# wljungbergh/mpc-trajectory-generator

Measured on AMD Instinct MI355X. Metric: nmpc_solves_per_sec, higher is better.
Workload: dtype f64

## Files before the change

### mpc_trajectory_generator_amd/csrc/nmpc_kernels.hip

```cpp
#include "nmpc_device.h"
#include "../../include/nmpc_solver.h"

#include <cfloat>
#include <cstdio>
#include <cstdlib>
#include <cstring>
#include <memory>
#include <string>
#include <vector>

#include "nmpc_layout.h"
#include "nmpc_probe.h"
#include "nmpc_eval.h"
#include "nmpc_solve_common.h"
#include "nmpc_solve_hyb.h"
#include "nmpc_solve_hyb2.h"
#include "nmpc_rng.h"
#include "nmpc_loop.h"
#include "nmpc_plan.h"
#include "nmpc_order.h"
#include "nmpc_host.h"

using nmpc::DevBuf;
using nmpc::Event;
// ... 18 lines not shown
    SOLVE_ROW(nmpc_solve_hyb_kernel, 20, Timed<ShapeNobs50>),
    SOLVE_ROW(nmpc_solve_hyb_kernel, 20, Timed<ShapeAny>),
    SOLVE_ROW(nmpc_solve_hyb2_kernel, 40, ShapeN40),
    SOLVE_ROW(nmpc_solve_hyb2_kernel, 40, ShapeAny),
    SOLVE_ROW(nmpc_solve_hyb2_kernel, 40, Timed<ShapeN40>),
    SOLVE_ROW(nmpc_solve_hyb2_kernel, 40, Timed<ShapeAny>),
};
#undef SOLVE_ROW
}
using nmpc::SolveKernel;

struct Staging {
    DevBuf<double> p, u, y0, c0, yout, psi, grad, F1, F2;
    DevBuf<nmpc_status> st;
    PinBuf pin[2];
    Event ev[2];
    bool ready = false;
};
struct SmallArena {
    DevBuf<char> d;
    PinBuf h;
    Event ev[2];
    bool ready = false;
    void release() { *this = {}; }
};
struct Pools {
    DevBuf<double> park;
    DevBuf<int> pool;
    DevBuf<unsigned int> ctr;
    bool made() const { return park && pool && ctr; }
    void release() { *this = {}; }
};

struct nmpc_handle {
    nmpc_problem pb{};
    nmpc_opts op{};
    int device = 0;
    int max_batch = 0;
    bool alive = true;
    LdsMap map{};
    int P = 20;
    const SolveKernel *kernel[2] = {nullptr, nullptr};
    int grid_cap = 0;
    double last_ms = 0.0;
    size_t team_lds = 0;
    size_t eval_lds = 0;
    DevBuf<unsigned int> d_queue;
    int park_min = 500, park_depth = 8;
    int sched_mode = 1;
    double sched_theta = 0.0, sched_cold = 0.4;
    bool shape_any = false;
    int team_owners_forced = 0;
    bool team_help = true;
    int waves_per_cu = 0;
    int dbg = 0;
    double cull_radius = 0.0;
    Pools pools;
    bool loop_order_prev = true;
    DevBuf<int> d_order;
    bool use_order = true;
    DevBuf<unsigned char> d_cls;
    Staging stg;
    SmallArena small;
    double tl_dur_ms = 0.0, tl_budget_ms = 0.0;
    long long tl_dur = 0, tl_budget = 0;
    DevBuf<long long> d_t0;
    std::string err;
};

__global__ void nmpc_stamp_kernel(long long *t0)
{
    if (threadIdx.x == 0) *t0 = (long long)__builtin_amdgcn_s_memrealtime();
}

extern "C" {

void nmpc_default_opts(nmpc_opts *o)
{
    o->tolerance = 1e-4;
    o->initial_tolerance = 1e-4;
    o->delta_tolerance = 1e-4;
    o->initial_penalty = 1.0;
    o->penalty_update = 5.0;
    o->tolerance_update = 0.1;
    o->sufficient_decrease = 0.1;
    o->lbfgs_memory = 10;
    o->max_inner = 500;
    o->max_outer = 10;
    o->max_total_inner = 0;
    o->akkt_gradient = 1;
    o->ls_failure = 0;
    o->inner_status = 0;
    o->reserved = 0;
}

int nmpc_n_u(const nmpc_problem *pb) { return 2 * pb->N; }
int nmpc_n1(const nmpc_problem *pb) { return 2 * pb->N; }
int nmpc_n2(const nmpc_problem *pb) { return pb->nobs + pb->ndyn; }
int nmpc_n_p(const nmpc_problem *pb) { return nmpc::NZ + pb->N + 3 * pb->nobs + 5 * pb->ndyn * pb->N + 3 * pb->N; }
int nmpc_abi_version(void) { return NMPC_ABI_VERSION; }
int nmpc_experiments_build(void)
{
#ifdef NMPC_EXPERIMENTS
    return 1;
#else
    return 0;
#endif
}

static int fail(nmpc_handle *h, int code, const char *what, hipError_t e = hipSuccess)
{
    if (h) {
        h->err = what;
        if (e != hipSuccess) { h->err += ": "; h->err += hipGetErrorString(e); }
    }
    return code;
}

#define HIP_TRY(h, call)                                                       \
    do {                                                                       \
        hipError_t e_ = (call);                                                \
        if (e_ != hipSuccess) return fail((h), NMPC_ERR_HIP, #call, e_);       \
    } while (0)

static constexpr size_t LDS_PER_CU = 160 * 1024;
static LdsMap make_map(const nmpc_problem &pb, int P) { return nmpc::lds_layout(pb.N, pb.nobs, pb.ndyn, P); }

static void read_knobs([[maybe_unused]] nmpc_handle *h)
{
#ifdef NMPC_EXPERIMENTS
    auto ival = [](const char *name, int &v) { if (const char *e = getenv(name)) v = atoi(e); };
    auto flag = [](const char *name, bool &v) { if (const char *e = getenv(name)) v = atoi(e) != 0; };
    auto pos = [](const char *name, double &v) { if (const char *e = getenv(name)) { const double x = atof(e); if (x > 0.0) v = x; } };
    if (const char *e = getenv("NMPC_SHAPE")) h->shape_any = !strcmp(e, "any");
    ival("NMPC_PARK_MIN", h->park_min);
    ival("NMPC_PARK_DEPTH", h->park_depth);
    flag("NMPC_LOOP_ORDER_PREV", h->loop_order_prev);
    ival("NMPC_SCHED", h->sched_mode);
    pos("NMPC_SCHED_THETA", h->sched_theta);
    pos("NMPC_SCHED_COLD", h->sched_cold);
    pos("NMPC_CULL_RADIUS", h->cull_radius);
    flag("NMPC_TEAM_HELP", h->team_help);
    flag("NMPC_ORDER", h->use_order);
    int owners = 0; ival("NMPC_TEAM_OWNERS", owners);
    if (owners >= 1 && owners <= nmpc::TEAM_WAVES) h->team_owners_forced = owners;
    ival("NMPC_WAVES_PER_CU", h->waves_per_cu);
    ival("NMPC_DEBUG_PRIO", h->dbg);
#endif
}

int nmpc_new(const nmpc_problem *pb, const nmpc_opts *opts, int device_id, int max_batch, nmpc_handle **out)
{
    if (!pb || !out || max_batch < 1) return NMPC_ERR_BAD_ARG;
    if (pb->N < 2 || pb->N > NMPC_MAX_HORIZON || pb->nobs < 0 || pb->nobs > 64 || pb->ndyn < 0 || pb->ndyn > nmpc::NDYN_MAX)
        return NMPC_ERR_BAD_PROBLEM;
    auto finite = [](double x) { return x >= -DBL_MAX && x <= DBL_MAX; };
    if (!(pb->ts > 0.0 && pb->ts <= DBL_MAX) || !finite(pb->vmin) || !finite(pb->vmax) || !(pb->vmin <= pb->vmax) ||
        !finite(pb->amin) || !finite(pb->amax) || !(pb->amin <= pb->amax) ||
        !(pb->wmax >= 0.0 && pb->wmax <= DBL_MAX) || !(pb->awmax >= 0.0 && pb->awmax <= DBL_MAX))
        return NMPC_ERR_BAD_PROBLEM;
    nmpc_opts op;
    if (opts) op = *opts; else nmpc_default_opts(&op);
    if (op.lbfgs_memory < 1 || op.lbfgs_memory > nmpc::MAXMEM || op.max_inner < 1 || op.max_outer < 1 ||
        op.max_total_inner < 0 || op.akkt_gradient < 0 || op.akkt_gradient > 2 || op.ls_failure < 0 || op.ls_failure > 1 ||
        op.inner_status < 0 || op.inner_status > 1)
        return NMPC_ERR_BAD_OPTS;
    auto finite_pos = [](double x) { return x > 0.0 && x <= DBL_MAX; };
    if (!finite_pos(op.tolerance) || !finite_pos(op.initial_tolerance) || !finite_pos(op.delta_tolerance) ||
        !(op.initial_tolerance >= op.tolerance) || !finite_pos(op.initial_penalty) ||
        !(op.penalty_update > 1.0 && op.penalty_update <= DBL_MAX) ||
        !(op.tolerance_update > 0.0 && op.tolerance_update < 1.0) ||
        !(op.sufficient_decrease > 0.0 && op.sufficient_decrease < 1.0))
        return NMPC_ERR_BAD_OPTS;
    int ndev = 0;
    if (hipGetDeviceCount(&ndev) != hipSuccess || ndev <= 0 || device_id < 0 || device_id >= ndev)
        return NMPC_ERR_NO_DEVICE;
    nmpc_handle *h = new nmpc_handle();
    h->pb = *pb; h->op = op; h->device = device_id; h->max_batch = max_batch;
    h->P = pb->N <= 20 ? 20 : 40;
    h->map = make_map(*pb, h->P == 40 ? 64 : h->P);
    h->sched_theta = h->P == 20 ? 0.5 : 0.8;
    h->cull_radius = 1.1 * pb->N * pb->ts * fmax(fabs(pb->vmin), fabs(pb->vmax));
    read_knobs(h);
    for (const SolveKernel &k : nmpc::SOLVE_KERNELS)
        if (k.P == h->P && (k.N == 0 ? !h->kernel[k.timed] : !h->shape_any && k.N == pb->N && k.nobs == pb->nobs && k.ndyn == pb->ndyn))
            h->kernel[k.timed] = &k;
    const size_t slice = (size_t)(h->P == 40 ? nmpc::lds_layout2(pb->N, pb->nobs, pb->ndyn).total : h->map.total) * sizeof(double);
    h->eval_lds = 3 * slice;
    h->team_lds = nmpc::TEAM_WAVES * slice + nmpc::TEAM_CTL_INTS * sizeof(int);
    if (h->eval_lds > LDS_PER_CU || h->team_lds > LDS_PER_CU) { nmpc_free(h); return NMPC_ERR_BAD_PROBLEM; }
    hipDeviceProp_t prop;
    hipError_t e = hipSetDevice(device_id);
    (void)hipGetDeviceProperties(&prop, device_id);
    if (e == hipSuccess) e = h->d_queue.alloc(1);
    if (e == hipSuccess) e = h->d_order.alloc(max_batch);
// ... 29 lines not shown
    const double t = ceil(ms * 1e5);
    const double cap = 4503599627370496.0;
    return t < 1.0 ? 1 : (long long)(t < cap ? t : cap);
}

int nmpc_set_time_limits(nmpc_handle *h, double max_duration_ms, double batch_budget_ms)
{
    if (!h) return NMPC_ERR_BAD_ARG;
    if (!h->alive) return NMPC_ERR_DEAD_HANDLE;
    auto ok = [](double x) { return x >= 0.0 && x <= DBL_MAX; };
    if (!ok(max_duration_ms) || !ok(batch_budget_ms)) return fail(h, NMPC_ERR_BAD_OPTS, "time limits: negative, NaN or infinite");
    const long long budget = ms_to_ticks(batch_budget_ms);
    if (budget > 0 && !h->d_t0) {
        HIP_TRY(h, hipSetDevice(h->device));
        HIP_TRY(h, h->d_t0.alloc(1));
    }
    h->tl_dur_ms = max_duration_ms; h->tl_budget_ms = batch_budget_ms;
    h->tl_dur = ms_to_ticks(max_duration_ms); h->tl_budget = budget;
    return NMPC_OK;
}

static int check_batch(nmpc_handle *h, int B, const double *p, const double *u)
{
    if (!h) return NMPC_ERR_BAD_ARG;
    if (!h->alive) return NMPC_ERR_DEAD_HANDLE;
    if (B < 0 || B > h->max_batch || (B > 0 && (!p || !u))) return fail(h, NMPC_ERR_BAD_ARG, "bad batch arguments");
    return NMPC_OK;
}

static void fill_args(const nmpc_handle *h, KArgs &a, int B)
{
    std::memset(&a, 0, sizeof(a));
    a.pb = h->pb; a.op = h->op; a.map = h->map; a.B = B;
    a.n_p = nmpc_n_p(&h->pb); a.n_u = nmpc_n_u(&h->pb); a.n1 = nmpc_n1(&h->pb); a.n2 = nmpc_n2(&h->pb);
    a.queue = h->d_queue;
    a.inv_ts = 1.0 / h->pb.ts;
    a.dbg = h->dbg;
    a.tl_dur = h->tl_dur; a.tl_budget = h->tl_budget;
    a.tl_t0 = h->tl_budget > 0 ? h->d_t0.p : nullptr;
}

static int solve_launch(nmpc_handle *h, int B, const double *d_p, double *d_u, const double *d_y0, const double *d_c0, double *d_y_out,
                        nmpc_status *d_status, const nmpc_status *prev, void *stream)
{
    if (const int rc = check_batch(h, B, d_p, d_u); rc || B == 0) return rc;
    hipStream_t s = (hipStream_t)stream;
    HIP_TRY(h, hipSetDevice(h->device));
    KArgs a;
    fill_args(h, a, B);
    a.p = d_p; a.u = d_u; a.y0 = d_y0; a.c0 = d_c0; a.y_out = d_y_out; a.st = d_status;
    if (h->tl_budget > 0) hipLaunchKernelGGL(nmpc_stamp_kernel, dim3(1), dim3(64), 0, s, h->d_t0.p);
    HIP_TRY(h, hipMemsetAsync(h->d_queue, 0, sizeof(unsigned int), s));
    const int grid = B < h->grid_cap ? B : h->grid_cap;
    if (B > grid) {
        if (h->use_order) {
            if (prev) hipLaunchKernelGGL(nmpc::nmpc_classify_prev_kernel, dim3((B + 255) / 256), dim3(256), 0, s, B, prev, h->d_cls.p);
            else hipLaunchKernelGGL(nmpc::nmpc_classify_kernel, dim3((B + 255) / 256), dim3(256), 0, s, a, h->d_cls.p);
            hipLaunchKernelGGL(nmpc::nmpc_order_kernel, dim3(1), dim3(1024), 0, s, B, h->d_cls.p, h->d_order.p);
            a.order = h->d_order;
        }
        if ((h->P == 20 && (h->park_min > 0 || h->sched_mode > 0)) || (h->P == 40 && h->sched_mode > 0)) {
            const size_t cap = (size_t)B;
            const size_t cap_max = (size_t)h->max_batch;
            Pools &pl = h->pools;
            if (!pl.made()) {
                pl.release();
                HIP_TRY(h, pl.park.alloc(cap_max * nmpc::park_stride(h->pb.N)));
                HIP_TRY(h, pl.pool.alloc(nmpc::NPOOLS * cap_max));
                HIP_TRY(h, pl.ctr.alloc(4 * nmpc::NPOOLS + 2));
            }
            HIP_TRY(h, hipMemsetAsync(pl.pool, 0xFF, nmpc::NPOOLS * cap * sizeof(int), s));
            HIP_TRY(h, hipMemsetAsync(pl.ctr, 0, (4 * nmpc::NPOOLS + 2) * sizeof(unsigned int), s));
            a.park_min = h->P == 20 ? h->park_min : 0; a.park_depth = h->park_depth;
            a.park = pl.park; a.pool = pl.pool; a.pool_ctr = pl.ctr; a.pool_cap = (int)cap;
            a.sched_mode = h->sched_mode;
        }
    }
    {
        const int max_wgs = h->grid_cap / nmpc::TEAM_WAVES;
        int owners = (B + max_wgs - 1) / max_wgs;
        if (owners > nmpc::TEAM_WAVES) owners = nmpc::TEAM_WAVES;
        if (h->team_owners_forced > 0) owners = h->team_owners_forced;
        int wgs = (grid + owners - 1) / owners;
        if (wgs > max_wgs) wgs = max_wgs;
        a.team_owners = owners;
        a.sched_long_cap = (int)(h->sched_theta * (double)(wgs * owners));
        a.sched_cold_cap = (int)(h->sched_cold * (double)(wgs * owners));
        a.team_help = h->team_help;
        a.cull_radius = h->cull_radius;
        hipLaunchKernelGGL(h->kernel[timed(h)]->fn, dim3(wgs), dim3(64 * nmpc::TEAM_WAVES), h->team_lds, s, a);
    }
    HIP_TRY(h, hipGetLastError());
    return NMPC_OK;
}

int nmpc_solve_batch_device(nmpc_handle *h, int B, const double *d_p, double *d_u, const double *d_y0,
                            const double *d_c0, double *d_y_out, nmpc_status *d_status, void *stream)
{
    return solve_launch(h, B, d_p, d_u, d_y0, d_c0, d_y_out, d_status, nullptr, stream);
}

int nmpc_eval_batch_device(nmpc_handle *h, int B, const double *d_p, const double *d_u, const double *d_c,
                           const double *d_y, double *d_psi, double *d_grad, double *d_F1, double *d_F2,
                           void *stream)
{
    if (const int rc = check_batch(h, B, d_p, d_u); rc || B == 0) return rc;
    hipStream_t s = (hipStream_t)stream;
    HIP_TRY(h, hipSetDevice(h->device));
    KArgs a;
    fill_args(h, a, B);
    a.p = d_p; a.u = const_cast<double *>(d_u);
    a.ev_c = d_c; a.ev_y = d_y; a.ev_psi = d_psi; a.ev_grad = d_grad; a.ev_F1 = d_F1; a.ev_F2 = d_F2;
    const dim3 grid((B + 2) / 3);
    if (h->P == 40) hipLaunchKernelGGL(nmpc::nmpc_eval2_kernel, grid, dim3(64), h->eval_lds, s, a);
    else hipLaunchKernelGGL(nmpc::nmpc_eval_kernel<20>, grid, dim3(64), h->eval_lds, s, a);
    HIP_TRY(h, hipGetLastError());
    return NMPC_OK;
}

static constexpr size_t PIN_CHUNK = 4u << 20;
static int ensure_staging(nmpc_handle *h)
{
    Staging &g = h->stg;
    if (g.ready) return NMPC_OK;
    if (g.p) return fail(h, NMPC_ERR_HIP, "staging buffers: an earlier allocation failed half way");
    const size_t B = (size_t)h->max_batch;
    const size_t np = nmpc_n_p(&h->pb), nu = nmpc_n_u(&h->pb), n1 = nmpc_n1(&h->pb), n2 = nmpc_n2(&h->pb) + 1;
    HIP_TRY(h, hipSetDevice(h->device));
    HIP_TRY(h, g.p.alloc(B * np));
    HIP_TRY(h, g.u.alloc(B * nu));
    HIP_TRY(h, g.y0.alloc(B * n1));
    HIP_TRY(h, g.c0.alloc(B));
    HIP_TRY(h, g.yout.alloc(B * n1));
    HIP_TRY(h, g.psi.alloc(B));
    HIP_TRY(h, g.grad.alloc(B * nu));
    HIP_TRY(h, g.F1.alloc(B * n1));
    HIP_TRY(h, g.F2.alloc(B * n2));
    HIP_TRY(h, g.st.alloc(B));
    for (int k = 0; k < 2; ++k) {
        HIP_TRY(h, g.pin[k].alloc(PIN_CHUNK));
        HIP_TRY(h, g.ev[k].create(hipEventDisableTiming));
    }
    g.ready = true;
    return NMPC_OK;
// ... 187 lines not shown
```

### mpc_trajectory_generator_amd/csrc/nmpc_layout.h

```cpp
#pragma once

#ifndef NMPC_WIN
#define NMPC_WIN 1
#endif

namespace nmpc {

constexpr int NZ = 20;
constexpr int MAXMEM = 10;
constexpr int NDYN_MAX = 3;
constexpr int GRAM_LD = 11;
constexpr int GRAM_NST = 20;
constexpr int OBS_STRIDE = 4;
constexpr int SEG_STRIDE = 5;
constexpr int TEAM_WAVES = 4;
constexpr int TEAM_REQ_DOUBLES = 3 * 24 * 2;
constexpr int TEAM_AREA_DOUBLES = 3 * 24 * 2 + 8;
constexpr int TEAM_CTL_INTS = 64;
constexpr int NPOOLS = 2;
enum { POOL_LONG = 0, POOL_COLD = 1 };

constexpr double GAMMA_L_COEFF = 0.95;
constexpr double DELTA_LIPSCHITZ = 1e-12;
constexpr double EPSILON_LIPSCHITZ = 1e-6;
constexpr double LIPSCHITZ_UPDATE_EPSILON = 1e-6;
constexpr int MAX_LIPSCHITZ_UPDATE_ITERATIONS = 10;
constexpr double MAX_LIPSCHITZ_CONSTANT = 1e9;
constexpr double MIN_LIPSCHITZ_CONSTANT = 1e-10;
constexpr int MAX_LINESEARCH_ITERATIONS = 10;
constexpr double LBFGS_SY_EPSILON = 1e-10;
constexpr double LBFGS_CBFGS_EPSILON = 1e-8;

struct LdsMap {
    int sc;
    int cw;
    int par;
    int seg;
    int obs;
    int f2;
    int dyn;
    int dyn_stride;
    int req;
    int vec;
    int rho;
    int S, Y;
    int nv;
    int gsy, gyy;
    int total;
};

struct KArgs {
    nmpc_problem pb;
    nmpc_opts op;
    LdsMap map;
    int B;
    int n_p, n_u, n1, n2;
    double inv_ts;
    const double *p;
    double *u;
    const double *y0;
    const double *c0;
    double *y_out;
    nmpc_status *st;
    unsigned int *queue;
    const int *order;
    int park_min;
    int park_depth;
    double *park;
    int *pool;
    unsigned int *pool_ctr;
    int pool_cap;
    int sched_mode;
    int sched_long_cap;
    int sched_cold_cap;
    int dbg;
    int team_owners;
    int team_help;
    double cull_radius;
    union {
        struct {
            const double *ev_c;
            const double *ev_y;
            double *ev_psi, *ev_grad, *ev_F1, *ev_F2;
        };
        struct {
            long long tl_dur;
            long long tl_budget;
            const long long *tl_t0;
        };
    };
};

enum { SC_X0 = 0, SC_Y0, SC_TH0, SC_VINIT, SC_WINIT, SC_XF, SC_YF, SC_THF,
       SC_Q, SC_QV, SC_QTH, SC_RV, SC_RW, SC_QN, SC_QTHN, SC_QCTE, SC_PA, SC_PW };

typedef __attribute__((address_space(3))) double lds_double;
typedef double dbl2 __attribute__((ext_vector_type(2)));
typedef __attribute__((address_space(3))) dbl2 lds_double2;

#ifdef NMPC_NO_SCHED_BARRIER
#define NMPC_SCHED_BARRIER() do { } while (0)
#else
#define NMPC_SCHED_BARRIER() __builtin_amdgcn_sched_barrier(0)
#endif
#define NMPC_WAVE_SYNC()                                           \
    do {                                                           \
        __builtin_amdgcn_fence(__ATOMIC_RELEASE, "workgroup");     \
        __builtin_amdgcn_wave_barrier();                           \
        __builtin_amdgcn_fence(__ATOMIC_ACQUIRE, "workgroup");     \
    } while (0)

enum { DY_EX = 0, DY_EY, DY_CA, DY_SA, DY_IRX2, DY_IRY2, DY_FIELDS };
struct DynStage {
    const lds_double *col;
    int stride;
    __device__ __forceinline__ double get(int k, int f) const { return col[(k * DY_FIELDS + f) * stride]; }
};

struct ShapeAny { static constexpr int N = 0, NOBS = -1, NDYN = -1; };
struct ShapeDefault { static constexpr int N = 20, NOBS = 10, NDYN = 3; };
struct ShapeNobs50 { static constexpr int N = 20, NOBS = 50, NDYN = 3; };
struct ShapeN40 { static constexpr int N = 40, NOBS = 10, NDYN = 3; };
template <class S> struct Timed { static constexpr int N = S::N, NOBS = S::NOBS, NDYN = S::NDYN; };
template <class SH> struct ShapeTimed { static constexpr bool value = false; };
template <class S> struct ShapeTimed<Timed<S>> { static constexpr bool value = true; };
template <class SH> __device__ __forceinline__ int shape_N(const KArgs &a) { if constexpr (SH::N > 0) return SH::N; else return a.pb.N; }
template <class SH> __device__ __forceinline__ int shape_nobs(const KArgs &a) { if constexpr (SH::NOBS >= 0) return SH::NOBS; else return a.pb.nobs; }
template <class SH> __device__ __forceinline__ int shape_ndyn(const KArgs &a) { if constexpr (SH::NDYN >= 0) return SH::NDYN; else return a.pb.ndyn; }

__host__ __device__ constexpr LdsMap lds_layout(int N, int nobs, int ndyn, int P)
// ... 103 lines not shown
```

### mpc_trajectory_generator_amd/csrc/nmpc_solve_hyb.h

```cpp
#pragma once

#ifndef NMPC_CULL_MIN
#define NMPC_CULL_MIN 16
#endif
#ifndef NMPC_WIN
#define NMPC_WIN 1
#endif

namespace nmpc {

typedef __attribute__((address_space(3))) int lds_int;
enum { CTL_OWNERS = 0, CTL_HELPERS = 1, CTL_CLAIM = 4, CTL_DONE = 8, CTL_INST = 56 };
__device__ __forceinline__ int ctl_load(lds_int *p) { return __hip_atomic_load(p, __ATOMIC_RELAXED, __HIP_MEMORY_SCOPE_WORKGROUP); }
__device__ __forceinline__ void ctl_store(lds_int *p, int v) { __hip_atomic_store(p, v, __ATOMIC_RELAXED, __HIP_MEMORY_SCOPE_WORKGROUP); }
__device__ __forceinline__ int ctl_add(lds_int *p, int v) { return __hip_atomic_fetch_add(p, v, __ATOMIC_RELAXED, __HIP_MEMORY_SCOPE_WORKGROUP); }

__device__ __forceinline__ double point_scalar(double v, int k)
{
    const int lo = __builtin_amdgcn_readlane(__double2loint(v), 16 * k);
    const int hi = __builtin_amdgcn_readlane(__double2hiint(v), 16 * k);
    return __hiloint2double(hi, lo);
}

#define NMPC_FETCH_GRAD(K, OV, OW)                                             \
    do {                                                                       \
        const dbl2 fg_ = zgr[(K) * ZS];                                        \
        OV = fg_.x; OW = fg_.y;                                                \
    } while (0)

#define NMPC_HALF_STEP(xv, xw)                                                 \
    do {                                                                       \
        const double s1_ = fma(-gamma, gv, (xv)), s2_ = fma(-gamma, gw, (xw)); \
        hv = ina ? clampd(s1_, vmin, vmax) : s1_;                              \
        hw = ina ? clampd(s2_, -wmax, wmax) : s2_;                             \
    } while (0)
#define NMPC_FBE(xv, xw) fbe_value<P>(cost, gamma, pk_hig, fma(-gamma, gv, (xv)), fma(-gamma, gw, (xw)), hv, hw, gv, gw, lane)

constexpr int POOL_CTRS = 4;
__device__ __forceinline__ int pool_pop(const KArgs &a, int c)
{
    unsigned int *ctr = a.pool_ctr + POOL_CTRS * c;
    int *cnt = (int *)(ctr + 2);
    if (__hip_atomic_load(cnt, __ATOMIC_RELAXED, __HIP_MEMORY_SCOPE_AGENT) <= 0) return -1;
    if (__hip_atomic_fetch_add(cnt, -1, __ATOMIC_RELAXED, __HIP_MEMORY_SCOPE_AGENT) <= 0) {
        __hip_atomic_fetch_add(cnt, 1, __ATOMIC_RELAXED, __HIP_MEMORY_SCOPE_AGENT);
        return -1;
    }
    const unsigned pos = __hip_atomic_fetch_add(&ctr[0], 1u, __ATOMIC_RELAXED, __HIP_MEMORY_SCOPE_AGENT);
    int *slot = a.pool + (size_t)c * a.pool_cap + pos % (unsigned)a.pool_cap;
    int inst;
    do { inst = __hip_atomic_load(slot, __ATOMIC_ACQUIRE, __HIP_MEMORY_SCOPE_AGENT); } while (inst < 0);
    __hip_atomic_store(slot, -1, __ATOMIC_RELAXED, __HIP_MEMORY_SCOPE_AGENT);
    return inst;
}
__device__ __forceinline__ void pool_push(const KArgs &a, int c, int inst)
{
    unsigned int *ctr = a.pool_ctr + POOL_CTRS * c;
    const unsigned pos = __hip_atomic_fetch_add(&ctr[1], 1u, __ATOMIC_RELAXED, __HIP_MEMORY_SCOPE_AGENT);
    int *slot = a.pool + (size_t)c * a.pool_cap + pos % (unsigned)a.pool_cap;
    while (__hip_atomic_load(slot, __ATOMIC_RELAXED, __HIP_MEMORY_SCOPE_AGENT) >= 0) __builtin_amdgcn_s_sleep(1);
    __hip_atomic_store(slot, inst, __ATOMIC_RELEASE, __HIP_MEMORY_SCOPE_AGENT);
    __hip_atomic_fetch_add((int *)(ctr + 2), 1, __ATOMIC_RELEASE, __HIP_MEMORY_SCOPE_AGENT);
}
__device__ __forceinline__ int pool_depth(const KArgs &a, int c)
{
    return __hip_atomic_load((int *)(a.pool_ctr + POOL_CTRS * c + 2), __ATOMIC_RELAXED, __HIP_MEMORY_SCOPE_AGENT);
}

template <int J>
__device__ __forceinline__ double fnma_row_bcast(double acc, double x, double y)
{
    asm("s_nop 1\n\tv_fmac_f64_dpp %0, -%1, %2 row_newbcast:%3 row_mask:0xf bank_mask:0xf" : "+v"(acc) : "v"(x), "v"(y), "n"(J));
    return acc;
}
template <int J>
__device__ __forceinline__ double fma_row_bcast(double acc, double x, double y)
{
    asm("s_nop 1\n\tv_fmac_f64_dpp %0, %1, %2 row_newbcast:%3 row_mask:0xf bank_mask:0xf" : "+v"(acc) : "v"(x), "v"(y), "n"(J));
    return acc;
}
template <int J>
__device__ __forceinline__ void fnma3_row_bcast(double &a1, double &a2, double &a3, double x, double y1, double y2, double y3, double after)
{
    asm("v_fmac_f64_dpp %0, -%3, %4 row_newbcast:%8 row_mask:0xf bank_mask:0xf\n\t"
        "v_fmac_f64_dpp %1, -%3, %5 row_newbcast:%8 row_mask:0xf bank_mask:0xf\n\t"
        "v_fmac_f64_dpp %2, -%3, %6 row_newbcast:%8 row_mask:0xf bank_mask:0xf"
        : "+v"(a1), "+v"(a2), "+v"(a3) : "v"(x), "v"(y1), "v"(y2), "v"(y3), "v"(after), "n"(J));
}
template <int J>
__device__ __forceinline__ void fma2_row_bcast(double &a1, double &a2, double x, double y1, double y2, double after)
{
// ... 166 lines not shown
    lds_double2 *Lgk = Los + 6 * COLS;
    lds_double2 *LypE = (lds_double2 *)(L + mp.vec) + 3 * COLS + te;
    lds_double2 *Ly = (lds_double2 *)(L + mp.vec) + 4 * COLS + te;
    lds_double *Lvr = L + mp.vec + 2 * 5 * COLS + te;
#define NMPC_LB_ZERO()                                                                                  \
    do {                                                                                                \
        lds_double2 *z_ = (lds_double2 *)(L + mp.gsy);                                                  \
        for (int i_ = lane; i_ < MAXMEM * GRAM_LD + 2 * MAXMEM * NS; i_ += 64) z_[i_] = dbl2{0.0, 0.0};  \
        if (lane < MAXMEM) Lrho[lane] = 0.0;                                                            \
    } while (0)
    if (threadIdx.x < TEAM_CTL_INTS) ctl[threadIdx.x] = threadIdx.x == CTL_OWNERS ? a.team_owners : 0;
    __syncthreads();
    lds_double2 *Lreq = (lds_double2 *)(L + mp.req);
    unsigned team_seq = 0;
    const double vmin = scalar_own(a.pb.vmin), vmax = scalar_own(a.pb.vmax), wmax = scalar_own(a.pb.wmax);
    const EvK ek = {scalar_own(a.pb.ts), scalar_own(a.inv_ts), scalar_own(a.pb.amin), scalar_own(a.pb.amax), scalar_own(a.pb.awmax)};
    const double tol_ = scalar_own(a.op.tolerance);
    const unsigned max_inner = (unsigned)scalar_own(a.op.max_inner);
    const unsigned budget = (unsigned)scalar_own(a.op.max_total_inner);
    constexpr bool TIMED = ShapeTimed<SH>::value;
    long long clk_batch = CLK_NEVER, clk_dl = CLK_NEVER;
    if constexpr (TIMED) { if (a.tl_budget > 0) clk_batch = uniform_ll(*a.tl_t0) + a.tl_budget; }
    lds_double *Lpar = L + mp.par;
#define pk_eps_nu Lpar[0]
#define pk_dy_norm Lpar[1]
#define pk_f2_norm Lpar[2]
#define pk_dy_norm_plus Lpar[3]
#define pk_f2_norm_plus Lpar[4]
#define pk_last_fpr Lpar[5]
#define pk_last_cost Lpar[6]
#define pk_norm_h Lpar[7]
#define pk_Lc Lpar[8]
#define pk_H0 Lpar[9]
#define pk_sigma Lpar[10]
#define pk_c_lip Lpar[11]
#define pk_fbe_u Lpar[20]
#define pk_hig Lpar[19]
#define pk_gr Lpar[12]


    const unsigned hw_slot = __builtin_amdgcn_s_getreg(((4 - 1) << 11) | (0 << 6) | 4);
    const bool unfavoured = hw_slot != 0u;
    const int PS = park_stride(N);

    const int n_waves = (int)gridDim.x * TEAM_WAVES;
    if (a.order && unfavoured && a.park_min > 0 && a.B >= n_waves + (n_waves >> 2)) {
        const unsigned want = (unsigned)n_waves / 2;
        const long long t_hold = (long long)__builtin_amdgcn_s_memrealtime();
        while (__hip_atomic_load(a.queue, __ATOMIC_RELAXED, __HIP_MEMORY_SCOPE_AGENT) < want &&
               (long long)__builtin_amdgcn_s_memrealtime() - t_hold < 4000)
            __builtin_amdgcn_s_sleep(8);
    }

    for (; wid < a.team_owners;) {
        int fetched = -1, from_pool = 0;
        if (lane == 0) {
            const bool pools = a.park_min > 0 || a.sched_mode > 0;
            if (pools && !unfavoured) { fetched = pool_pop(a, POOL_LONG); from_pool = fetched >= 0; }
            if (fetched < 0) {
                const unsigned nxt = atomicAdd(a.queue, 1u);
                if (nxt < (unsigned)a.B) fetched = a.order ? a.order[nxt] : (int)nxt;
                else if (pools) {
                    for (int c = 0; c < NPOOLS && fetched < 0; ++c) fetched = pool_pop(a, c);
                    from_pool = fetched >= 0;
                }
            }
        }
        const int inst = __builtin_amdgcn_readfirstlane(fetched);
        const bool resumed = __builtin_amdgcn_readfirstlane(from_pool) != 0;
        if (inst < 0) break;

        const long long dbg_t0 = __builtin_amdgcn_s_memtime();
        const auto clk0_ = __builtin_amdgcn_s_memrealtime();
        long long t_first = (long long)clk0_;
        Lpar[13] = (double)clk0_; Lpar[14] = 0.0;
        if (k_dbg == 1) { if (hw_slot & 1u) __builtin_amdgcn_s_setprio(0); else __builtin_amdgcn_s_setprio(3); }
        double vref_;
        DynStage dyn;
        if (lane == 0) ctl_store(ctl + CTL_INST + wid, -1);
        __builtin_amdgcn_fence(__ATOMIC_RELEASE, "workgroup");
        prepare_instance<PE, SH>(a, L, a.p + (size_t)inst * a.n_p, te, vref_, dyn);
        *Lvr = vref_;
        WinState ws = {te < N - 1 ? te : N - 2, 0.0, 0.0, 0.0};
        ObsCert oc = {0.0, 0.0, 0.0, 0, 0, 0};
        __builtin_amdgcn_fence(__ATOMIC_RELEASE, "workgroup");
        if (lane == 0) ctl_store(ctl + CTL_INST + wid, inst);
        unsigned long long near = ~0ull;
        if constexpr (CULL) {
            near = circle_near_mask(a.p + (size_t)inst * a.n_p, N, shape_nobs<SH>(a), lane, a.cull_radius);
            if (lane == 0) { Lpar[18] = __hiloint2double((int)(near >> 32), (int)near); }
        }

        const double *pk = a.park + (size_t)inst * PS;
        const double *u0 = resumed ? pk : a.u + (size_t)inst * a.n_u;
        double uv = in ? u0[2 * t] : 0.0, uw = in ? u0[2 * t + 1] : 0.0;
        {
            double yv0, yw0;
            if (resumed) {
                yv0 = ine ? pk[2 * N + 2 * te] : 0.0;
                yw0 = ine ? pk[2 * N + 2 * te + 1] : 0.0;
            } else {
                yv0 = (a.y0 && ine) ? a.y0[(size_t)inst * a.n1 + te] : 0.0;
                yw0 = (a.y0 && ine) ? a.y0[(size_t)inst * a.n1 + N + te] : 0.0;
            }
            *LypE = dbl2{yv0, yw0};
            *Ly = dbl2{yv0, yw0};
        }
        *Lq = (resumed && in) ? dbl2{pk[4 * N + 2 * t], pk[4 * N + 2 * t + 1]} : dbl2{0.0, 0.0};
        double gv = 0, gw = 0, hv = 0, hw = 0, rv = 0, rw = 0, dv = 0, dw = 0;
        unsigned fl = 0u;
        FlagBit need_grad{fl, 1u << 0}; need_grad = true;
        double cost = 0, gamma = 0, tau = 1, rhs_ls = 0;
        pk_fbe_u = 0.0; pk_hig = 0.0;
        pk_Lc = 0.0; pk_sigma = 0.0; pk_H0 = 1.0;
        FlagBit fbe_ok{fl, 1u << 1};
        int iteration = 0, lip_it = 0, ls_n = 0, lb_active = 0, lb_head = 0;
        FlagBit lb_first{fl, 1u << 2}; lb_first = true;
// ... 420 lines not shown
                                gv = in ? prev_g.x : 0.0; gw = in ? prev_g.y : 0.0;
                            }
                            NMPC_TL_KEEP(uv + pv + gv + hv); NMPC_TL_EV(tl_it, 10);
                            posted = false;
                            if (lane == 0) ctl_store(ctl + CTL_CLAIM + wid, 0);
                        }
                        if (rejected) f_trials = true;
                        else if (exhausted) f_fb = true;
                        else { uv = pv; uw = pw; pk_fbe_u = lhs; fbe_ok = true; NMPC_END_ITERATION(); }
                    }
                }
            } else if (state == D_LS) {
                NMPC_TAKE_TRIAL(psiA, src0);
                if (rejected) NMPC_TAKE_TRIAL(psiB, src1);
                if (rejected) NMPC_TAKE_TRIAL(psiC, src2);
                if (rejected) f_trials = true;
                else if (exhausted) f_fb = true;
                else { uv = pv; uw = pw; pk_fbe_u = lhs; fbe_ok = true; NMPC_END_ITERATION(); }
            } else if (state == D_FB) {
                n_grad++;
                uv = hv; uw = hw;
                cost = psiA;
                NMPC_FETCH_GRAD(src0, gv, gw);
                NMPC_HALF_STEP(uv, uw);
                fbe_ok = false;
                NMPC_END_ITERATION();
            } else {
                n_cost++;
                const double tv = fma(yv, cbar_inv, eav), tw = fma(yw, cbar_inv, eaw);
                const double ypv = inea ? fma(pen_c, eav - clampd(tv, ek.amin, ek.amax), yv) : 0.0;
                const double ypw = inea ? fma(pen_c, eaw - clampd(tw, -ek.awmax, ek.awmax), yw) : 0.0;
                *LypE = dbl2{ypv, ypw};
                const double d1 = ypv - yv, d2 = ypw - yw;
                pk_dy_norm_plus = sqrt(group_sum<PE>(inea ? fma(d1, d1, d2 * d2) : 0.0, lane));
                pk_f2_norm_plus = sqrt(pen);
                const double SMALL = DBL_EPSILON;
                const bool crit1 = nu > 0 && __any(pk_dy_norm_plus <= pen_c * a.op.delta_tolerance + SMALL);
                const bool crit2 = a.n2 == 0 || __any(pk_f2_norm_plus <= a.op.delta_tolerance + SMALL);
                const bool crit3 = __any(pk_eps_nu <= a.op.tolerance + SMALL);
                if (crit1 && crit2 && crit3) {
                    final_status = a.op.inner_status == 1 ? NMPC_CONVERGED : inner_status; running = false;
                } else {
                    const bool stall = nu == 0 || __any(pk_dy_norm_plus <= a.op.sufficient_decrease * pk_dy_norm + SMALL &&
                                                        pk_f2_norm_plus <= a.op.sufficient_decrease * pk_f2_norm + SMALL);
                    if (!stall) { pen_c *= a.op.penalty_update; cbar_inv = 1.0 / fmax(pen_c, 1.0); }
                    pk_eps_nu = fmax(a.op.tolerance_update * pk_eps_nu, a.op.tolerance);
                    *Ly = dbl2{ypv, ypw};
                    pk_dy_norm = pk_dy_norm_plus; pk_f2_norm = pk_f2_norm_plus;
                    nu++;
                    if (nu == a.op.max_outer) { final_status = NMPC_NOT_CONVERGED_ITERATIONS; running = false; }
                    else if (timed_out) { final_status = NMPC_NOT_CONVERGED_OUT_OF_TIME; running = false; nu--; }
                    else {
                        bool yield_ = false;
                        if (a.sched_mode > 0 || a.park_min > 0) {
                            int dec = 0;
                            if (lane == 0) {
                                const bool fresh_left = (int)__hip_atomic_load(a.queue, __ATOMIC_RELAXED, __HIP_MEMORY_SCOPE_AGENT) < a.B;
                                int cls = POOL_LONG, y = 0;
                                if (a.sched_mode > 0) {
                                    const bool long_now = !(crit2 && pk_dy_norm_plus <= pen_c * a.op.delta_tolerance + SMALL);
                                    cls = long_now ? POOL_LONG : POOL_COLD;
                                    unsigned int *n_long = a.pool_ctr + POOL_CTRS * NPOOLS;
                                    if (long_now != long_counted) __hip_atomic_fetch_add(n_long, long_now ? 1u : ~0u, __ATOMIC_RELAXED, __HIP_MEMORY_SCOPE_AGENT);
                                    const bool long_wait = pool_depth(a, POOL_LONG) > 0;
                                    const int alive = (int)__hip_atomic_load(n_long, __ATOMIC_RELAXED, __HIP_MEMORY_SCOPE_AGENT);
                                    if (cls == POOL_COLD) y = (fresh_left || long_wait) && alive >= a.sched_cold_cap && n_pass >= 150u;
                                    else y = (fresh_left || long_wait) && alive >= a.sched_long_cap && n_pass - q_pass >= 150u;
                                    dec = (long_now ? 2 : 0);
                                }
                                if (!y && a.park_min > 0 && unfavoured && n_pass >= (unsigned)a.park_min && fresh_left && pool_depth(a, POOL_LONG) < a.park_depth) {
                                    y = 1; cls = POOL_LONG;
                                }
                                dec |= y | (cls << 2);
                            }
                            dec = __builtin_amdgcn_readfirstlane(dec);
                            yield_ = (dec & 1) != 0;
                            if (a.sched_mode > 0) long_counted = (dec & 2) != 0;
                            park_cls = dec >> 2;
                        }
                        q_pass = n_pass;
                        if (yield_) { parked = true; running = false; }
                        else f_start = true;
                    }
                }
            }
            NMPC_SEC_KEEP(uv + gv + hv + cost);
            NMPC_SEC(6);
        }

        if (parked) {
            double *po = a.park + (size_t)inst * PS;
            if (in && h == 0) {
                po[2 * t] = uv; po[2 * t + 1] = uw;
                const dbl2 q_ = *Lq;
                po[4 * N + 2 * t] = q_.x; po[4 * N + 2 * t + 1] = q_.y;
            }
            if (ine && q == 0) { const dbl2 y_ = *Ly; po[2 * N + 2 * te] = y_.x; po[2 * N + 2 * te + 1] = y_.y; }
            if (lane == 0) {
                double *ps_ = po + 6 * N;
                ps_[0] = pen_c; ps_[1] = pk_eps_nu; ps_[2] = pk_dy_norm; ps_[3] = pk_f2_norm; ps_[4] = pk_dy_norm_plus;
                ps_[5] = pk_f2_norm_plus; ps_[6] = pk_last_fpr; ps_[7] = pk_last_cost; ps_[8] = (double)nu;
                ps_[9] = (double)inner_total; ps_[10] = (double)n_cost; ps_[11] = (double)n_grad; ps_[12] = (double)n_pass;
                ps_[13] = Lpar[13]; ps_[14] = Lpar[14]; ps_[15] = long_counted ? 1.0 : 0.0;
            }
            __builtin_amdgcn_fence(__ATOMIC_RELEASE, "agent");
            __builtin_amdgcn_wave_barrier();
            if (lane == 0) pool_push(a, park_cls, inst);
            if (k_dbg == 0) __builtin_amdgcn_s_setprio(0);
            NMPC_WAVE_SYNC();
            continue;
        }
        if (in && h == 0) {
            double *uo = a.u + (size_t)inst * a.n_u;
            uo[2 * t] = uv; uo[2 * t + 1] = uw;
            if (a.y_out) { const dbl2 yp_ = *Lyp; a.y_out[(size_t)inst * a.n1 + t] = yp_.x; a.y_out[(size_t)inst * a.n1 + N + t] = yp_.y; }
        }
        if (lane == 0 && long_counted) __hip_atomic_fetch_add(a.pool_ctr + POOL_CTRS * NPOOLS, ~0u, __ATOMIC_RELAXED, __HIP_MEMORY_SCOPE_AGENT);
        if (lane == 0 && a.st) {
            nmpc_status s;
            s.exit_status = final_status;
            s.num_outer_iterations = (uint32_t)(final_status == NMPC_NOT_CONVERGED_NOT_FINITE ? nu + 1 : (nu < a.op.max_outer ? nu + 1 : nu));
            s.num_inner_iterations = inner_total;
            s.num_cost_evals = n_cost;
            s.num_grad_evals = n_grad;
            s.reserved = n_pass;
            s.last_problem_norm_fpr = pk_last_fpr;
            s.delta_y_norm_over_c = pk_dy_norm_plus / pen_c;
            s.f2_norm = pk_f2_norm_plus;
            s.penalty = pen_c;
            s.cost = pk_last_cost;
            s.solve_time_ms = (double)((long long)__builtin_amdgcn_s_memrealtime() - (long long)Lpar[13]) * 1e-5;
            if (k_dbg) {
                s.last_problem_norm_fpr = (double)(__builtin_amdgcn_s_memtime() - dbg_t0);
                s.f2_norm = (double)hw_slot;
                s.cost = (double)__builtin_amdgcn_s_memrealtime();
                s.delta_y_norm_over_c = Lpar[13]; s.penalty = Lpar[14];
            }
            NMPC_PROBE_STATUS(s);
            a.st[inst] = s;
        }
        if (k_dbg == 0) __builtin_amdgcn_s_setprio(0);
        NMPC_WAVE_SYNC();
    }

    if (k_dbg == 0) __builtin_amdgcn_s_setprio(0);
    if (lane == 0) ctl_store(ctl + CTL_INST + wid, -1);
    __builtin_amdgcn_fence(__ATOMIC_RELEASE, "workgroup");
    if (lane == 0) {
        if (wid < a.team_owners) ctl_add(ctl + CTL_OWNERS, -1);
        ctl_add(ctl + CTL_HELPERS, 1);
    }
    WinState ws_h = {te < N - 1 ? te : N - 2, 0.0, 0.0, 0.0};
    ObsCert oc_h = {0.0, 0.0, 0.0, 0, 0, 0};
    int ws_inst = -1;
    for (;;) {
        if (!k_help || __builtin_amdgcn_readfirstlane(ctl_load(ctl + CTL_OWNERS)) <= 0) break;
        int got = -1;
        if (lane == 0) {
            for (int w = 0; w < TEAM_WAVES && got < 0; ++w) {
                if (w == wid) continue;
                int v = ctl_load(ctl + CTL_CLAIM + w);
                if ((v >> 8) != 0 && (v & 0xff) < 3 &&
                    __hip_atomic_compare_exchange_strong(ctl + CTL_CLAIM + w, &v, v + 1, __ATOMIC_RELAXED, __ATOMIC_RELAXED,
                                                         __HIP_MEMORY_SCOPE_WORKGROUP))
                    got = (w << 28) | (v & 0x0fffffff);
            }
        }
        got = __builtin_amdgcn_readfirstlane(got);
        if (got < 0) { __builtin_amdgcn_s_sleep(2); continue; }
        const int w = got >> 28, k = got & 0xff;
        NMPC_TL_HELPER((lds_double *)lds + w * slice, k)
        NMPC_TL_EV(tl_h, 11);
        const int seq = (got & 0x0fffffff) >> 8;
        __builtin_amdgcn_fence(__ATOMIC_ACQUIRE, "workgroup");
        lds_double *Lw = (lds_double *)lds + w * slice;
        const lds_double2 *rq = (const lds_double2 *)(Lw + mp.req) + te;
        const dbl2 u_ = rq[0], r_ = rq[24], d_ = rq[48];
        const double c_w = Lw[mp.par + 15], cbar_w = Lw[mp.par + 16];
        const dbl2 y_w = ((const lds_double2 *)(Lw + mp.vec) + 4 * COLS)[te];
        const double vref_w = Lw[mp.vec + 2 * 5 * COLS + te];
        DynStage dyn_w;
        dyn_w.col = Lw + mp.dyn + te;
        dyn_w.stride = lay_cols<PE>();
        const double tau_w = __hiloint2double((1023 - (2 + 3 * k + q)) << 20, 0), omt_w = 1.0 - tau_w;
        const double zv = fma(-tau_w, d_.x, fma(-omt_w, r_.x, u_.x)), zw = fma(-tau_w, d_.y, fma(-omt_w, r_.y, u_.y));
        double psi, pen, egv = 0, egw = 0, eav, eaw;
        unsigned long long near_w = ~0ull;
        if constexpr (CULL) { const double nb_ = Lw[mp.par + 18]; near_w = ((unsigned long long)(unsigned)__double2hiint(nb_) << 32) | (unsigned)__double2loint(nb_); }
        {
            const int inst_w = __builtin_amdgcn_readfirstlane(ctl_load(ctl + CTL_INST + w));
            __builtin_amdgcn_fence(__ATOMIC_ACQUIRE, "workgroup");
            if (inst_w != ws_inst || inst_w < 0) { ws_inst = inst_w; ws_h.mo2 = 0.0; oc_h.m2 = 0.0; }
        }
        NMPC_TL_KEEP(zv + zw); NMPC_TL_EV(tl_h, 12);
        eval_psi<PE, SH, false, CULL, WIN>(a, Lw, f2off, lane, te, zv, zw, c_w, cbar_w, y_w.x, y_w.y, vref_w, dyn_w, true, psi, pen, egv, egw, eav, eaw, near_w, &ws_h, OBSC ? &oc_h : nullptr, nullptr, &ek);
        NMPC_TL_KEEP(psi + egv); NMPC_TL_EV(tl_h, 13);
        {
            __builtin_amdgcn_fence(__ATOMIC_ACQUIRE, "workgroup");
            if (__builtin_amdgcn_readfirstlane(ctl_load(ctl + CTL_INST + w)) != ws_inst) { ws_inst = -1; ws_h.mo2 = 0.0; oc_h.m2 = 0.0; }
        }
        const double gam_w = Lw[mp.par + 17], hig_w = Lw[mp.par + 19];
        const double s1_ = fma(-gam_w, egv, zv), s2_ = fma(-gam_w, egw, zw);
        const double e1_ = s1_ - (inea ? clampd(s1_, vmin, vmax) : s1_), e2_ = s2_ - (inea ? clampd(s2_, -wmax, wmax) : s2_);
        const double dist2_ = group_sum<PE>(inea ? fma(e1_, e1_, e2_ * e2_) : 0.0, lane);
        const double gg_ = group_sum<PE>(inea ? fma(egv, egv, egw * egw) : 0.0, lane);
        const double lhs_ = psi - (0.5 * gam_w) * gg_ + dist2_ * hig_w;
        lds_double *ar = L + (w * 3 + k) * TEAM_AREA_DOUBLES;
        ((lds_double2 *)ar)[24 * q + te] = dbl2{egv, egw};
        if (te == 0) { ar[2 * 72 + q] = psi; ar[2 * 72 + 4 + q] = lhs_; }
// ... 36 lines not shown
```

Measured before the change: 229,800.

## Add tail-team pool so idle workgroups absorb long-running solves at batch end

Adds a third pool (POOL_TAIL) and global counters so that, once the fresh queue is drained, a workgroup whose owners are busy can hand a long-running instance to a workgroup whose owners all ran out of work. That workgroup's last owner spins waiting on the tail pool instead of exiting, and its helpers keep waiting until all instances are finished. The aim is to cut the tail-latency imbalance where a few hard instances keep one workgroup's waves busy while other CUs sit idle. In exchange it adds global atomics, polling loops with sleeps, park/unpark state traffic, and changes to the owner-count bookkeeping, which risks deadlock or contention.

```diff
diff --git a/mpc_trajectory_generator_amd/csrc/nmpc_kernels.hip b/mpc_trajectory_generator_amd/csrc/nmpc_kernels.hip
--- a/mpc_trajectory_generator_amd/csrc/nmpc_kernels.hip
+++ b/mpc_trajectory_generator_amd/csrc/nmpc_kernels.hip
@@ -94,6 +94,7 @@
     bool shape_any = false;
     int team_owners_forced = 0;
     bool team_help = true;
+    bool tail_teams = true;
     int waves_per_cu = 0;
     int dbg = 0;
     double cull_radius = 0.0;
@@ -183,6 +184,7 @@
     pos("NMPC_SCHED_COLD", h->sched_cold);
     pos("NMPC_CULL_RADIUS", h->cull_radius);
     flag("NMPC_TEAM_HELP", h->team_help);
+    flag("NMPC_TAIL_TEAMS", h->tail_teams);
     flag("NMPC_ORDER", h->use_order);
     int owners = 0; ival("NMPC_TEAM_OWNERS", owners);
     if (owners >= 1 && owners <= nmpc::TEAM_WAVES) h->team_owners_forced = owners;
@@ -318,44 +320,46 @@
     if (h->tl_budget > 0) hipLaunchKernelGGL(nmpc_stamp_kernel, dim3(1), dim3(64), 0, s, h->d_t0.p);
     HIP_TRY(h, hipMemsetAsync(h->d_queue, 0, sizeof(unsigned int), s));
     const int grid = B < h->grid_cap ? B : h->grid_cap;
-    if (B > grid) {
-        if (h->use_order) {
-            if (prev) hipLaunchKernelGGL(nmpc::nmpc_classify_prev_kernel, dim3((B + 255) / 256), dim3(256), 0, s, B, prev, h->d_cls.p);
-            else hipLaunchKernelGGL(nmpc::nmpc_classify_kernel, dim3((B + 255) / 256), dim3(256), 0, s, a, h->d_cls.p);
-            hipLaunchKernelGGL(nmpc::nmpc_order_kernel, dim3(1), dim3(1024), 0, s, B, h->d_cls.p, h->d_order.p);
-            a.order = h->d_order;
+    const int max_wgs = h->grid_cap / nmpc::TEAM_WAVES;
+    int owners = (B + max_wgs - 1) / max_wgs;
+    if (owners > nmpc::TEAM_WAVES) owners = nmpc::TEAM_WAVES;
+    if (h->team_owners_forced > 0) owners = h->team_owners_forced;
+    int wgs = (grid + owners - 1) / owners;
+    if (wgs > max_wgs) wgs = max_wgs;
+    const bool tail = h->tail_teams && h->P == 20 && owners >= 2 && h->team_help;
+    if (B > grid && h->use_order) {
+        if (prev) hipLaunchKernelGGL(nmpc::nmpc_classify_prev_kernel, dim3((B + 255) / 256), dim3(256), 0, s, B, prev, h->d_cls.p);
+        else hipLaunchKernelGGL(nmpc::nmpc_classify_kernel, dim3((B + 255) / 256), dim3(256), 0, s, a, h->d_cls.p);
+        hipLaunchKernelGGL(nmpc::nmpc_order_kernel, dim3(1), dim3(1024), 0, s, B, h->d_cls.p, h->d_order.p);
+        a.order = h->d_order;
+    }
+    const bool sched = B > grid && ((h->P == 20 && (h->park_min > 0 || h->sched_mode > 0)) || (h->P == 40 && h->sched_mode > 0));
+    if (sched || tail) {
+        const size_t cap = (size_t)B;
+        const size_t cap_max = (size_t)h->max_batch;
+        constexpr size_t n_ctr = 4 * nmpc::NPOOLS + nmpc::POOL_EXTRA_CTRS;
+        Pools &pl = h->pools;
+        if (!pl.made()) {
+            pl.release();
+            HIP_TRY(h, pl.park.alloc(cap_max * nmpc::park_stride(h->pb.N)));
+            HIP_TRY(h, pl.pool.alloc(nmpc::NPOOLS * cap_max));
+            HIP_TRY(h, pl.ctr.alloc(n_ctr));
         }
-        if ((h->P == 20 && (h->park_min > 0 || h->sched_mode > 0)) || (h->P == 40 && h->sched_mode > 0)) {
-            const size_t cap = (size_t)B;
-            const size_t cap_max = (size_t)h->max_batch;
-            Pools &pl = h->pools;
-            if (!pl.made()) {
-                pl.release();
-                HIP_TRY(h, pl.park.alloc(cap_max * nmpc::park_stride(h->pb.N)));
-                HIP_TRY(h, pl.pool.alloc(nmpc::NPOOLS * cap_max));
-                HIP_TRY(h, pl.ctr.alloc(4 * nmpc::NPOOLS + 2));
-            }
-            HIP_TRY(h, hipMemsetAsync(pl.pool, 0xFF, nmpc::NPOOLS * cap * sizeof(int), s));
-            HIP_TRY(h, hipMemsetAsync(pl.ctr, 0, (4 * nmpc::NPOOLS + 2) * sizeof(unsigned int), s));
+        HIP_TRY(h, hipMemsetAsync(pl.pool, 0xFF, nmpc::NPOOLS * cap * sizeof(int), s));
+        HIP_TRY(h, hipMemsetAsync(pl.ctr, 0, n_ctr * sizeof(unsigned int), s));
+        a.park = pl.park; a.pool = pl.pool; a.pool_ctr = pl.ctr; a.pool_cap = (int)cap;
+        if (sched) {
             a.park_min = h->P == 20 ? h->park_min : 0; a.park_depth = h->park_depth;
-            a.park = pl.park; a.pool = pl.pool; a.pool_ctr = pl.ctr; a.pool_cap = (int)cap;
             a.sched_mode = h->sched_mode;
         }
-    }
-    {
-        const int max_wgs = h->grid_cap / nmpc::TEAM_WAVES;
-        int owners = (B + max_wgs - 1) / max_wgs;
-        if (owners > nmpc::TEAM_WAVES) owners = nmpc::TEAM_WAVES;
-        if (h->team_owners_forced > 0) owners = h->team_owners_forced;
-        int wgs = (grid + owners - 1) / owners;
-        if (wgs > max_wgs) wgs = max_wgs;
-        a.team_owners = owners;
-        a.sched_long_cap = (int)(h->sched_theta * (double)(wgs * owners));
-        a.sched_cold_cap = (int)(h->sched_cold * (double)(wgs * owners));
-        a.team_help = h->team_help;
-        a.cull_radius = h->cull_radius;
-        hipLaunchKernelGGL(h->kernel[timed(h)]->fn, dim3(wgs), dim3(64 * nmpc::TEAM_WAVES), h->team_lds, s, a);
-    }
+        a.tail_teams = tail;
+    }
+    a.team_owners = owners;
+    a.sched_long_cap = (int)(h->sched_theta * (double)(wgs * owners));
+    a.sched_cold_cap = (int)(h->sched_cold * (double)(wgs * owners));
+    a.team_help = h->team_help;
+    a.cull_radius = h->cull_radius;
+    hipLaunchKernelGGL(h->kernel[timed(h)]->fn, dim3(wgs), dim3(64 * nmpc::TEAM_WAVES), h->team_lds, s, a);
     HIP_TRY(h, hipGetLastError());
     return NMPC_OK;
 }
diff --git a/mpc_trajectory_generator_amd/csrc/nmpc_layout.h b/mpc_trajectory_generator_amd/csrc/nmpc_layout.h
--- a/mpc_trajectory_generator_amd/csrc/nmpc_layout.h
+++ b/mpc_trajectory_generator_amd/csrc/nmpc_layout.h
@@ -17,8 +17,10 @@
 constexpr int TEAM_REQ_DOUBLES = 3 * 24 * 2;
 constexpr int TEAM_AREA_DOUBLES = 3 * 24 * 2 + 8;
 constexpr int TEAM_CTL_INTS = 64;
-constexpr int NPOOLS = 2;
-enum { POOL_LONG = 0, POOL_COLD = 1 };
+constexpr int NPOOLS = 3;
+enum { POOL_LONG = 0, POOL_COLD = 1, POOL_TAIL = 2 };
+constexpr int POOL_EXTRA_CTRS = 4;
+enum { XC_LONG = 0, XC_TEAMS_WAITING = 1, XC_FINISHED = 2 };
 
 constexpr double GAMMA_L_COEFF = 0.95;
 constexpr double DELTA_LIPSCHITZ = 1e-12;
@@ -76,6 +78,7 @@
     int dbg;
     int team_owners;
     int team_help;
+    int tail_teams;
     double cull_radius;
     union {
         struct {
diff --git a/mpc_trajectory_generator_amd/csrc/nmpc_solve_hyb.h b/mpc_trajectory_generator_amd/csrc/nmpc_solve_hyb.h
--- a/mpc_trajectory_generator_amd/csrc/nmpc_solve_hyb.h
+++ b/mpc_trajectory_generator_amd/csrc/nmpc_solve_hyb.h
@@ -10,7 +10,7 @@
 namespace nmpc {
 
 typedef __attribute__((address_space(3))) int lds_int;
-enum { CTL_OWNERS = 0, CTL_HELPERS = 1, CTL_CLAIM = 4, CTL_DONE = 8, CTL_INST = 56 };
+enum { CTL_OWNERS = 0, CTL_HELPERS = 1, CTL_OVER = 2, CTL_CLAIM = 4, CTL_DONE = 8, CTL_INST = 56 };
 __device__ __forceinline__ int ctl_load(lds_int *p) { return __hip_atomic_load(p, __ATOMIC_RELAXED, __HIP_MEMORY_SCOPE_WORKGROUP); }
 __device__ __forceinline__ void ctl_store(lds_int *p, int v) { __hip_atomic_store(p, v, __ATOMIC_RELAXED, __HIP_MEMORY_SCOPE_WORKGROUP); }
 __device__ __forceinline__ int ctl_add(lds_int *p, int v) { return __hip_atomic_fetch_add(p, v, __ATOMIC_RELAXED, __HIP_MEMORY_SCOPE_WORKGROUP); }
@@ -37,6 +37,7 @@
 #define NMPC_FBE(xv, xw) fbe_value<P>(cost, gamma, pk_hig, fma(-gamma, gv, (xv)), fma(-gamma, gw, (xw)), hv, hw, gv, gw, lane)
 
 constexpr int POOL_CTRS = 4;
+__device__ __forceinline__ unsigned int *extra_ctr(const KArgs &a, int which) { return a.pool_ctr + POOL_CTRS * NPOOLS + which; }
 __device__ __forceinline__ int pool_pop(const KArgs &a, int c)
 {
     unsigned int *ctr = a.pool_ctr + POOL_CTRS * c;
@@ -309,10 +310,11 @@
             __builtin_amdgcn_s_sleep(8);
     }
 
+    bool gave_away = false;
     for (; wid < a.team_owners;) {
         int fetched = -1, from_pool = 0;
-        if (lane == 0) {
-            const bool pools = a.park_min > 0 || a.sched_mode > 0;
+        if (lane == 0 && !gave_away) {
+            const bool pools = a.park_min > 0 || a.sched_mode > 0 || a.tail_teams;
             if (pools && !unfavoured) { fetched = pool_pop(a, POOL_LONG); from_pool = fetched >= 0; }
             if (fetched < 0) {
                 const unsigned nxt = atomicAdd(a.queue, 1u);
@@ -320,6 +322,20 @@
                 else if (pools) {
                     for (int c = 0; c < NPOOLS && fetched < 0; ++c) fetched = pool_pop(a, c);
                     from_pool = fetched >= 0;
+                }
+            }
+            if (fetched < 0) {
+                if (ctl_add(ctl + CTL_OWNERS, -1) == 1 && a.tail_teams) {
+                    __hip_atomic_fetch_add(extra_ctr(a, XC_TEAMS_WAITING), 1u, __ATOMIC_RELAXED, __HIP_MEMORY_SCOPE_AGENT);
+                    for (;;) {
+                        if (__hip_atomic_load(extra_ctr(a, XC_FINISHED), __ATOMIC_RELAXED, __HIP_MEMORY_SCOPE_AGENT) >= (unsigned)a.B) {
+                            ctl_store(ctl + CTL_OVER, 1);
+                            break;
+                        }
+                        if ((fetched = pool_pop(a, POOL_TAIL)) >= 0) { from_pool = 1; ctl_add(ctl + CTL_OWNERS, 1); break; }
+                        for (int i = 0; i < 8; ++i) __builtin_amdgcn_s_sleep(127);
+                    }
+                    __hip_atomic_fetch_add(extra_ctr(a, XC_TEAMS_WAITING), ~0u, __ATOMIC_RELAXED, __HIP_MEMORY_SCOPE_AGENT);
                 }
             }
         }
@@ -846,7 +862,7 @@
                     else if (timed_out) { final_status = NMPC_NOT_CONVERGED_OUT_OF_TIME; running = false; nu--; }
                     else {
                         bool yield_ = false;
-                        if (a.sched_mode > 0 || a.park_min > 0) {
+                        if (a.sched_mode > 0 || a.park_min > 0 || a.tail_teams) {
                             int dec = 0;
                             if (lane == 0) {
                                 const bool fresh_left = (int)__hip_atomic_load(a.queue, __ATOMIC_RELAXED, __HIP_MEMORY_SCOPE_AGENT) < a.B;
@@ -865,6 +881,14 @@
                                 if (!y && a.park_min > 0 && unfavoured && n_pass >= (unsigned)a.park_min && fresh_left && pool_depth(a, POOL_LONG) < a.park_depth) {
                                     y = 1; cls = POOL_LONG;
                                 }
+                                if (!y && a.tail_teams && !fresh_left && n_pass - q_pass >= 150u &&
+                                    (int)__hip_atomic_load(extra_ctr(a, XC_TEAMS_WAITING), __ATOMIC_RELAXED, __HIP_MEMORY_SCOPE_AGENT) > pool_depth(a, POOL_TAIL)) {
+                                    int v = ctl_load(ctl + CTL_OWNERS);
+                                    if (v >= 2 && __hip_atomic_compare_exchange_strong(ctl + CTL_OWNERS, &v, v - 1, __ATOMIC_RELAXED, __ATOMIC_RELAXED,
+                                                                                       __HIP_MEMORY_SCOPE_WORKGROUP)) {
+                                        y = 1; cls = POOL_TAIL;
+                                    }
+                                }
                                 dec |= y | (cls << 2);
                             }
                             dec = __builtin_amdgcn_readfirstlane(dec);
@@ -895,13 +919,15 @@
                 ps_[0] = pen_c; ps_[1] = pk_eps_nu; ps_[2] = pk_dy_norm; ps_[3] = pk_f2_norm; ps_[4] = pk_dy_norm_plus;
                 ps_[5] = pk_f2_norm_plus; ps_[6] = pk_last_fpr; ps_[7] = pk_last_cost; ps_[8] = (double)nu;
                 ps_[9] = (double)inner_total; ps_[10] = (double)n_cost; ps_[11] = (double)n_grad; ps_[12] = (double)n_pass;
-                ps_[13] = Lpar[13]; ps_[14] = Lpar[14]; ps_[15] = long_counted ? 1.0 : 0.0;
+                ps_[13] = Lpar[13]; ps_[14] = Lpar[14] + (park_cls == POOL_TAIL ? 1024.0 : 0.0);
+                ps_[15] = long_counted ? 1.0 : 0.0;
             }
             __builtin_amdgcn_fence(__ATOMIC_RELEASE, "agent");
             __builtin_amdgcn_wave_barrier();
             if (lane == 0) pool_push(a, park_cls, inst);
             if (k_dbg == 0) __builtin_amdgcn_s_setprio(0);
             NMPC_WAVE_SYNC();
+            if (park_cls == POOL_TAIL) gave_away = true;
             continue;
         }
         if (in && h == 0) {
@@ -910,6 +936,7 @@
             if (a.y_out) { const dbl2 yp_ = *Lyp; a.y_out[(size_t)inst * a.n1 + t] = yp_.x; a.y_out[(size_t)inst * a.n1 + N + t] = yp_.y; }
         }
         if (lane == 0 && long_counted) __hip_atomic_fetch_add(a.pool_ctr + POOL_CTRS * NPOOLS, ~0u, __ATOMIC_RELAXED, __HIP_MEMORY_SCOPE_AGENT);
+        if (lane == 0 && a.tail_teams) __hip_atomic_fetch_add(extra_ctr(a, XC_FINISHED), 1u, __ATOMIC_RELAXED, __HIP_MEMORY_SCOPE_AGENT);
         if (lane == 0 && a.st) {
             nmpc_status s;
             s.exit_status = final_status;
@@ -926,7 +953,7 @@
             s.solve_time_ms = (double)((long long)__builtin_amdgcn_s_memrealtime() - (long long)Lpar[13]) * 1e-5;
             if (k_dbg) {
                 s.last_problem_norm_fpr = (double)(__builtin_amdgcn_s_memtime() - dbg_t0);
-                s.f2_norm = (double)hw_slot;
+                s.f2_norm = (double)(hw_slot + 16u * (unsigned)wid + 64u * blockIdx.x);
                 s.cost = (double)__builtin_amdgcn_s_memrealtime();
                 s.delta_y_norm_over_c = Lpar[13]; s.penalty = Lpar[14];
             }
@@ -940,15 +967,17 @@
     if (k_dbg == 0) __builtin_amdgcn_s_setprio(0);
     if (lane == 0) ctl_store(ctl + CTL_INST + wid, -1);
     __builtin_amdgcn_fence(__ATOMIC_RELEASE, "workgroup");
-    if (lane == 0) {
-        if (wid < a.team_owners) ctl_add(ctl + CTL_OWNERS, -1);
-        ctl_add(ctl + CTL_HELPERS, 1);
-    }
+    if (lane == 0) ctl_add(ctl + CTL_HELPERS, 1);
     WinState ws_h = {te < N - 1 ? te : N - 2, 0.0, 0.0, 0.0};
     ObsCert oc_h = {0.0, 0.0, 0.0, 0, 0, 0};
     int ws_inst = -1;
     for (;;) {
-        if (!k_help || __builtin_amdgcn_readfirstlane(ctl_load(ctl + CTL_OWNERS)) <= 0) break;
+        if (!k_help) break;
+        if (__builtin_amdgcn_readfirstlane(ctl_load(ctl + CTL_OWNERS)) <= 0) {
+            if (!a.tail_teams || __builtin_amdgcn_readfirstlane(ctl_load(ctl + CTL_OVER)) != 0) break;
+            for (int i = 0; i < 8; ++i) __builtin_amdgcn_s_sleep(127);
+            continue;
+        }
         int got = -1;
         if (lane == 0) {
             for (int w = 0; w < TEAM_WAVES && got < 0; ++w) {
```

Measured after the change: 230,800, median of 4. About the same (+0.4%).
